# CVMI-Lab/HybridNeuralRendering

Hardware: AMD Instinct MI355X
Metric: rays/sec (fwd render) scene0241_01 at 1/2/4/8 GPU; PSNR delta vs ref (higher is better)
Workload: dtype f32

## Files before the change

### hybridneuralrendering_amd/csrc/mlp.hip

```cpp
#include <stdlib.h>

#include "hnr_h2.h"
#include "hnr_launch.h"

namespace hnr {

constexpr int ML_PAD = 32;
constexpr int ML_SLOT = 8192 + ML_PAD;
constexpr int ML_WSTEP = 8192;
constexpr int ML_META_FLOATS = 4 * 128 + 4 + 4;
constexpr int ML_DESC = 4 * 128, ML_WMAX = 4 * 128 + 4;

struct MlpArgs {
    const float *A; int lda;
    const float *R; const int32_t *ridx; int ldr;
    const char *wimg;
    int wbase[4];
    int K0, N[4], act[4];
    float *C2; int ldc2;
    const float *loc_w; const int32_t *vs_item;
    const float *w2c, *Kmat, *campos, *campos_n;
    const float *fm; int H, W;
    const float *frame_w;
    const float *w_last, *b_last;
    const float *CF; int ldcf;
    float *X7; int ld7;
    float slope;
    const unsigned long long *counts; int count_index, count_mult; long long M_cap;
    int seg_stride;
    float *C; int ldc;
    float *T0; int ldt0; float *T1; int ldt1;
    unsigned *tmax;
};

typedef float f32x4m __attribute__((ext_vector_type(4)));

#ifdef HNR_MLP_PROBE
__device__ long long g_mlp_probe[24];
#define MLP_STAMP(i_) do { const long long t_ = clock64(); tm_[i_] += t_ - tp_; tp_ = t_; if ((i_) == 0) ++ntile_; } while (0)
#else
#define MLP_STAMP(i_) do { } while (0)
#endif
constexpr int mlp3_wgs_per_cu(int S0, int RT, int MODE) { return MODE == 1 ? (RT >= 4 ? 2 : 4) : RT >= 4 ? 1 : (RT == 1 || S0 <= 6) ? 4 : 2; }

#ifdef HNR_MLP_FULL_BARRIER
#define MLP_LDS_BARRIER() __syncthreads()
#else
#define MLP_LDS_BARRIER() asm volatile("s_waitcnt lgkmcnt(0)\n\ts_barrier" ::: "memory")
#endif
#ifndef HNR_MLP_LPR16
#define HNR_MLP_LPR16 1
#endif
template <int S0, int S1, int S2, int S3, int MODE, int RT = 4>
__global__ __launch_bounds__(256, mlp3_wgs_per_cu(S0, RT, MODE)) void mlp3_kernel(MlpArgs a)
{
    static_assert(MODE != 1 || RT == 4 || RT == 2, "the merge stage is built on 128- or 64-row tiles (32 / 16 samples x 4 views)");
    constexpr int SLOT = RT * 2048 + ML_PAD, ROWS = 32 * RT;
    constexpr int SMAX3 = S0 > S1 ? (S0 > S2 ? S0 : S2) : (S1 > S2 ? S1 : S2), SMAX = SMAX3 > S3 ? SMAX3 : S3;
    extern __shared__ __attribute__((aligned(16))) char lds[];
    const int tid = threadIdx.x, lane = tid & 63, wave = tid >> 6, h = lane >> 5, j = lane & 31;
    long long M = a.M_cap;
    if (a.counts) { const long long c = (long long)a.counts[a.count_index] * a.count_mult; if (c < M) M = c; }
    long long n_unit = 1;
    if (a.seg_stride > 0) {
        n_unit = a.counts ? (long long)a.counts[a.count_index] : a.M_cap / (a.count_mult > 0 ? a.count_mult : 1);
        if (n_unit > a.seg_stride) n_unit = a.seg_stride;
        if (n_unit < 1) n_unit = 1;
        if (M > n_unit * a.count_mult) M = n_unit * a.count_mult;
    }
    auto phys = [&](long long m) -> long long {
        if (a.seg_stride <= 0) return m;
        int q = 0;
        for (int v = 1; v < a.count_mult && v < 8; ++v) q += (m >= (long long)v * n_unit) ? 1 : 0;
        return (long long)q * a.seg_stride + (m - (long long)q * n_unit);
    };
    const int n_tiles = (int)((M + ROWS - 1) / ROWS);
    const int total_steps = S0 + S1 + S2 + S3;
    const float *meta = reinterpret_cast<const float *>(a.wimg + (size_t)total_steps * ML_WSTEP);
    const __amdgpu_buffer_rsrc_t wsrd = __builtin_amdgcn_make_buffer_rsrc(const_cast<char *>(a.wimg), 0, total_steps * ML_WSTEP, 0x00020000);
    float *exch = reinterpret_cast<float *>(lds + SMAX * SLOT);
    float *rowinv = exch + ROWS * 4;
    float *s_f = rowinv + ROWS;
    int *s_pix = reinterpret_cast<int *>(s_f + ROWS * 48);
    float *s_vm = reinterpret_cast<float *>(s_pix + ROWS), *s_w = s_vm + ROWS;
    float *s_wl = s_w + ROWS;
    constexpr bool RS = S1 <= 4 && S2 <= 4 && S3 == 0 && RT >= 2;
    constexpr int RTW = RS ? RT / 2 : RT;
    const int cw = RS ? (wave & 1) : wave, rt0 = RS ? (wave >> 1) * RTW : 0;
    const int col0 = 32 * cw + 16 * h;
    const unsigned woff = (unsigned)cw * 2048u + (unsigned)lane * 16u;
    const char *lds_b = lds + rt0 * 2048;
    const f32x2 slope2 = {a.slope, a.slope};

    if (MODE == 1) {
        for (int i = tid; i < 128; i += 256) s_wl[i] = i < a.N[2] ? a.w_last[i] : 0.f;
    }
    float tmax_run[3] = {0.f, 0.f, 0.f};
#ifdef HNR_MLP_PROBE
    long long tm_[20] = {0, 0, 0, 0, 0, 0, 0, 0, 0, 0, 0, 0, 0, 0, 0, 0, 0, 0, 0, 0}, tp_ = clock64(), ntile_ = 0;
#endif
    for (int tile = blockIdx.x; tile < n_tiles; tile += gridDim.x) {
        const long long row_base = (long long)tile * ROWS;
        int tid_t = tid;
        asm volatile("" : "+v"(tid_t));
        MLP_STAMP(0);
        float inv[RTW];
        if (MODE == 1) {
            if (tid < 2 * ROWS) {
                const int row_t = tid % ROWS, ls = row_t >> 2, v = row_t & 3;
                long long sidx = row_base / 4 + ls;
                if (sidx * 4 >= M) sidx = M / 4 - 1;
                const float *pw = a.loc_w + (size_t)a.vs_item[sidx] * 3;
                const float x = pw[0], y = pw[1], z = pw[2];
              if (tid < ROWS) {
                int px, py;
                const bool inval = hnr_project_pixel(x, y, z, a.w2c + 16 * v, a.Kmat, a.W, a.H, px, py);
                s_pix[tid] = ((v * a.H + py) * a.W + px) * 48;
                s_vm[tid] = inval ? 0.f : 1.f;
              } else {
                const float cx = x - a.campos[0], cy = y - a.campos[1], cz = z - a.campos[2];
                const float cn = sqrtf(cx * cx + cy * cy + cz * cz) + 1e-6f;
                const float nx = x - a.campos_n[3 * v], ny = y - a.campos_n[3 * v + 1], nz = z - a.campos_n[3 * v + 2];
                const float nn = sqrtf(nx * nx + ny * ny + nz * nz) + 1e-6f;
                s_f[row_t * 48 + 45] = hnr_div(nx, nn) - hnr_div(cx, cn); s_f[row_t * 48 + 46] = hnr_div(ny, nn) - hnr_div(cy, cn); s_f[row_t * 48 + 47] = hnr_div(nz, nn) - hnr_div(cz, cn);
              }
            }
            MLP_STAMP(13);
            __syncthreads();
            {
                constexpr int NF = ROWS * 12 / 256;
                float4 f4[NF];
#pragma unroll
                for (int it = 0; it < NF; ++it) {
                    const int idx = tid_t + 256 * it, row = idx / 12, q = idx - row * 12;
                    f4[it] = *reinterpret_cast<const float4 *>(a.fm + (size_t)s_pix[row] + 4 * q);
                }
#pragma unroll
                for (int it = 0; it < NF; ++it) {
                    const int idx = tid_t + 256 * it, row = idx / 12, q = idx - row * 12;
                    float *d = s_f + row * 48 + 4 * q;
                    if (q < 11) *reinterpret_cast<float4 *>(d) = f4[it]; else d[0] = f4[it].x;
                }
            }
            __syncthreads();
            if (wave < RT) {
                const float *src = s_f + (32 * wave + j) * 48 + 8 * h;
                float x[3][8];
                float m = 0.f;
#pragma unroll
                for (int s = 0; s < 3; ++s) {
                    const float4 v0 = *reinterpret_cast<const float4 *>(src + 16 * s), v1 = *reinterpret_cast<const float4 *>(src + 16 * s + 4);
                    const float t[8] = {v0.x, v0.y, v0.z, v0.w, v1.x, v1.y, v1.z, v1.w};
#pragma unroll
                    for (int e = 0; e < 8; ++e) { x[s][e] = t[e]; m = fmaxf(m, fabsf(t[e])); }
                }
                m = fmaxf(m, __shfl_xor(m, 32));
                const int k = row_scale_exp(m);
                const float sc = pow2f(k);
                if (h == 0) rowinv[32 * wave + j] = pow2f(-k);
#pragma unroll
                for (int s = 0; s < 3; ++s) {
                    unsigned ph[4], pm[4];
#pragma unroll
                    for (int q = 0; q < 4; ++q) split2h(__fmul_rn(x[s][2 * q], sc), __fmul_rn(x[s][2 * q + 1], sc), ph[q], pm[q]);
                    char *dst = lds + s * SLOT + (wave * 2) * 1024 + lane * 16;
                    *reinterpret_cast<u32x4 *>(dst) = u32x4{ph[0], ph[1], ph[2], ph[3]};
                    *reinterpret_cast<u32x4 *>(dst + 1024) = u32x4{pm[0], pm[1], pm[2], pm[3]};
                }
            }
        } else
        {
            constexpr int COLS = 16 * S0, LPR = HNR_MLP_LPR16 && COLS == 288 ? 16 : (COLS > 128 ? 64 : (COLS > 64 ? 32 : 16)), RPI = 64 / LPR, NB = (COLS + 4 * LPR - 1) / (4 * LPR);
            const int lr = lane % LPR, sub = lane / LPR;
            constexpr int RW = 8 * RT;
            constexpr int ROWS_B = ((RW / RPI) * NB * 4 <= (RT < 4 ? 128 : 256)) ? RW : RW / 2;
            constexpr int BATCH = ROWS_B / RPI;
#pragma unroll 1
            for (int r0 = 0; r0 < RW; r0 += ROWS_B) {
                float4 v[BATCH][NB];
#pragma unroll
                for (int b = 0; b < BATCH; ++b) {
                    const int rl = RW * wave + r0 + b * RPI + sub;
                    long long row = row_base + rl;
                    if (row >= M) row = M - 1;
                    const float *src = a.A + (size_t)phys(row) * a.lda;
#pragma unroll
                    for (int nb = 0; nb < NB; ++nb) {
                        const int c = 4 * (nb * LPR + lr);
                        v[b][nb] = *reinterpret_cast<const float4 *>(src + (c + 4 <= a.lda ? c : 0));
                    }
                }
#pragma unroll
                for (int b = 0; b < BATCH; ++b) {
                    const int rl = RW * wave + r0 + b * RPI + sub;
                    float m = 0.f;
#pragma unroll
                    for (int nb = 0; nb < NB; ++nb) {
                        const int c = 4 * (nb * LPR + lr);
                        float *t = reinterpret_cast<float *>(&v[b][nb]);
#pragma unroll
                        for (int e = 0; e < 4; ++e) { t[e] = (c + e < a.K0) ? t[e] : 0.f; m = fmaxf(m, fabsf(t[e])); }
                    }
                    m = fmaxf(m, __builtin_amdgcn_update_dpp(m, m, 0xB1, 0xf, 0xf, false));
                    m = fmaxf(m, __builtin_amdgcn_update_dpp(m, m, 0x4E, 0xf, 0xf, false));
                    m = fmaxf(m, __builtin_amdgcn_update_dpp(m, m, 0x141, 0xf, 0xf, false));
                    m = fmaxf(m, __builtin_amdgcn_update_dpp(m, m, 0x140, 0xf, 0xf, false));
                    if (LPR >= 32) m = fmaxf(m, __builtin_amdgcn_update_dpp(m, m, 0x142, 0xa, 0xf, false));
                    if (LPR >= 64) m = fmaxf(m, __builtin_amdgcn_update_dpp(m, m, 0x143, 0xc, 0xf, false));
                    if (LPR == 64) m = __int_as_float(__builtin_amdgcn_readlane(__float_as_int(m), 63));
                    else if (LPR == 32) { const float m0 = __int_as_float(__builtin_amdgcn_readlane(__float_as_int(m), 31)), m1 = __int_as_float(__builtin_amdgcn_readlane(__float_as_int(m), 63)); m = sub ? m1 : m0; }
                    const int k = row_scale_exp(m);
                    const float sc = pow2f(k);
                    if (lr == 0) rowinv[rl] = pow2f(-k);
#pragma unroll
                    for (int nb = 0; nb < NB; ++nb) {
                        const int c = 4 * (nb * LPR + lr);
                        if (c < COLS) {
                            unsigned ph0, pm0, ph1, pm1;
                            split2h(__fmul_rn(v[b][nb].x, sc), __fmul_rn(v[b][nb].y, sc), ph0, pm0);
                            split2h(__fmul_rn(v[b][nb].z, sc), __fmul_rn(v[b][nb].w, sc), ph1, pm1);
                            char *dst = lds + (c >> 4) * SLOT + ((rl >> 5) * 2) * 1024 + ((((c >> 3) & 1) * 32 + (rl & 31)) * 16) + (c & 7) * 2;
                            *reinterpret_cast<uint2 *>(dst) = make_uint2(ph0, ph1);
                            *reinterpret_cast<uint2 *>(dst + 1024) = make_uint2(pm0, pm1);
                        }
                    }
                }
            }
        }
        MLP_STAMP(1);
        __syncthreads();
        MLP_STAMP(2);
        {
            const float dw0 = meta[ML_DESC + 0];
#pragma unroll
            for (int rt = 0; rt < RTW; ++rt) inv[rt] = __fmul_rn(rowinv[32 * (rt0 + rt) + j], dw0);
        }

        f32x16 acc[RTW][1];
        auto zero_acc = [&]() {
#pragma unroll
            for (int rt = 0; rt < RTW; ++rt)
#pragma unroll
                for (int r = 0; r < 16; ++r) acc[rt][0][r] = 0.f;
        };
        float4 ad[2][4];
        auto load_addend = [&](int rt) {
            long long row = row_base + 32 * (rt0 + rt) + j;
            if (row >= M) row = M - 1;
            const float *rrow = a.R + (size_t)(MODE == 1 ? row / 4 : (long long)a.ridx[phys(row)]) * a.ldr + col0;
#pragma unroll
            for (int q4 = 0; q4 < 4; ++q4) ad[rt & 1][q4] = *reinterpret_cast<const float4 *>(rrow + 4 * q4);
        };
        auto activate = [&](int layer, float (&amax)[RTW], auto with_addend) {
            constexpr bool ADD = decltype(with_addend)::value;
            f32x2 bias[8];
#pragma unroll
            for (int q = 0; q < 4; ++q) {
                const float4 b = *reinterpret_cast<const float4 *>(meta + layer * 128 + col0 + 4 * q);
                bias[2 * q] = f32x2{b.x, b.y}; bias[2 * q + 1] = f32x2{b.z, b.w};
            }
            const bool act = a.act[layer] != 0;
            if (ADD && MODE != 1) { load_addend(0); if (RTW > 1) load_addend(1); }
#pragma unroll
            for (int rt = 0; rt < RTW; ++rt) {
                float m = 0.f;
                const f32x2 inv2 = {inv[rt], inv[rt]};
#pragma unroll
                for (int q = 0; q < 8; ++q) {
                    f32x2 add = bias[q];
                    if (ADD) { const float4 t4 = ad[rt & 1][q >> 1]; add = add + ((q & 1) ? f32x2{t4.z, t4.w} : f32x2{t4.x, t4.y}); }
                    f32x2 v = f32x2_fma(f32x2{acc[rt][0][2 * q], acc[rt][0][2 * q + 1]}, inv2, add);
                    if (act) { const f32x2 sv = v * slope2; v.x = fmaxf(v.x, sv.x); v.y = fmaxf(v.y, sv.y); }
                    acc[rt][0][2 * q] = v.x; acc[rt][0][2 * q + 1] = v.y;
                    m = fmaxf(fmaxf(m, fabsf(v.x)), fabsf(v.y));
                }
                amax[rt] = m;
                if (ADD && rt + 2 < RTW) load_addend(rt + 2);
            }
        };
        auto publish = [&](int next_layer, bool active, float (&amax)[RTW]) {
#pragma unroll
            for (int rt = 0; rt < RTW; ++rt) {
                const float m = active ? fmaxf(amax[rt], __shfl_xor(amax[rt], 32)) : 0.f;
                if (h == 0) exch[(32 * (rt0 + rt) + j) * 4 + cw] = m;
            }
            __syncthreads();
            const float dw = meta[ML_DESC + next_layer];
#pragma unroll
            for (int rt = 0; rt < RTW; ++rt) {
                float4 m4 = *reinterpret_cast<const float4 *>(exch + (32 * (rt0 + rt) + j) * 4);
                if (RS) { m4.z = 0.f; m4.w = 0.f; }
                const int k = row_scale_exp(fmaxf(fmaxf(m4.x, m4.y), fmaxf(m4.z, m4.w)));
                const float sc = pow2f(k);
                const f32x2 sc2 = {sc, sc};
                inv[rt] = __fmul_rn(pow2f(-k), dw);
                if (active) {
                    unsigned ph[8], pm[8];
#pragma unroll
                    for (int q = 0; q < 8; ++q) {
                        const f32x2 vs = f32x2{acc[rt][0][2 * q], acc[rt][0][2 * q + 1]} * sc2;
                        split2h(vs.x, vs.y, ph[q], pm[q]);
                    }
                    char *dst = lds + (2 * cw + h) * SLOT + ((rt0 + rt) * 2) * 1024 + j * 16;
                    *reinterpret_cast<u32x4 *>(dst) = u32x4{ph[0], ph[1], ph[2], ph[3]};
                    *reinterpret_cast<u32x4 *>(dst + 512) = u32x4{ph[4], ph[5], ph[6], ph[7]};
                    *reinterpret_cast<u32x4 *>(dst + 1024) = u32x4{pm[0], pm[1], pm[2], pm[3]};
                    *reinterpret_cast<u32x4 *>(dst + 1024 + 512) = u32x4{pm[4], pm[5], pm[6], pm[7]};
                }
            }
            __syncthreads();
        };
        auto store = [&](float *C, int ldc) {
#pragma unroll
            for (int rt = 0; rt < RTW; ++rt) {
                const long long row = row_base + 32 * (rt0 + rt) + j;
                if (row < M) {
                    float *o = C + (size_t)phys(row) * ldc + col0;
#pragma unroll
                    for (int q = 0; q < 4; ++q) {
                        const int c = col0 + 4 * q;
                        if (c + 4 <= ldc)
                            *reinterpret_cast<float4 *>(o + 4 * q) = make_float4(acc[rt][0][4 * q], acc[rt][0][4 * q + 1], acc[rt][0][4 * q + 2], acc[rt][0][4 * q + 3]);
                    }
                }
            }
        };
        const bool act0 = 32 * cw < a.N[0], act1 = 32 * cw < a.N[1], act2 = 32 * cw < a.N[2];
        float amax[RTW];
        zero_acc();
        if (act0) {
            h2_mfma_layer<RTW, 1, S0, 0, ML_WSTEP, SLOT>(wsrd, a.wbase[0], woff, lds_b, lane, acc, []() {}, [&]() { if (MODE == 1) { load_addend(0); load_addend(1); } });
            MLP_STAMP(3);
            if (a.R) activate(0, amax, std::true_type{}); else activate(0, amax, std::false_type{});
            MLP_STAMP(4);
            if (MODE == 0 && a.T0) {
                store(a.T0, a.ldt0);
#pragma unroll
                for (int rt = 0; rt < RTW; ++rt) tmax_run[0] = fmaxf(tmax_run[0], amax[rt]);
            }
        }
        publish(1, act0, amax);
        MLP_STAMP(5);
        zero_acc();
        if (act1) {
            h2_mfma_layer<RTW, 1, S1, 0, ML_WSTEP, SLOT>(wsrd, a.wbase[1], woff, lds_b, lane, acc, []() {});
            MLP_STAMP(6);
            activate(1, amax, std::false_type{});
            if (MODE == 0 && a.T1) {
                store(a.T1, a.ldt1);
#pragma unroll
                for (int rt = 0; rt < RTW; ++rt) tmax_run[1] = fmaxf(tmax_run[1], amax[rt]);
            }
        }
        publish(2, act1, amax);
        MLP_STAMP(7);
        float cfv[6] = {0.f, 0.f, 0.f, 0.f, 0.f, 0.f};
        float4 wl4[4];
        zero_acc();
        if (act2) {
            h2_mfma_layer<RTW, 1, S2, 0, ML_WSTEP, SLOT>(wsrd, a.wbase[2], woff, lds_b, lane, acc, []() {});
            MLP_STAMP(8);
            activate(2, amax, std::false_type{});
            MLP_STAMP(9);
            if (MODE != 1) store(a.C, a.ldc);
            if (MODE == 0 && a.tmax) {
#pragma unroll
                for (int rt = 0; rt < RTW; ++rt) tmax_run[2] = fmaxf(tmax_run[2], amax[rt]);
            }
            MLP_STAMP(10);
        }
        if (MODE == 1) {
#pragma unroll
            for (int it = 0; it < (8 * RT * 45 + 255) / 256; ++it) {
                const int idx = tid_t + 256 * it, ls = idx / 45, ch = idx - ls * 45;
                const long long sidx = row_base / 4 + ls;
                cfv[it] = (idx < 8 * RT * 45 && sidx * 4 < M) ? a.CF[(size_t)sidx * a.ldcf + ch] : 0.f;
            }
#pragma unroll
            for (int q4 = 0; q4 < 4; ++q4) wl4[q4] = *reinterpret_cast<const float4 *>(s_wl + col0 + 4 * q4);
        }
        if (MODE == 1) {
#pragma unroll
            for (int rt = 0; rt < RTW; ++rt) {
                float d = 0.f;
                if (act2) {
#pragma unroll
                    for (int r = 0; r < 16; ++r) d = fmaf(acc[rt][0][r], reinterpret_cast<const float *>(wl4)[r], d);
                    d = __fadd_rn(d, __shfl_xor(d, 32));
                }
                if (h == 0) exch[(32 * (rt0 + rt) + j) * 4 + cw] = d;
            }
            MLP_LDS_BARRIER();
            MLP_STAMP(14);
            if (tid < ROWS) {
                float4 d4 = *reinterpret_cast<const float4 *>(exch + tid * 4);
                if (RS) { d4.z = 0.f; d4.w = 0.f; }
                const float d = __fadd_rn(__fadd_rn(d4.x, d4.y), __fadd_rn(d4.z, d4.w));
                float wv = hnr_div(1.f, 1.f + expf(-(d + a.b_last[0])));
                wv *= s_vm[tid];
                if (a.frame_w) wv *= a.frame_w[tid & 3];
                s_w[tid] = wv;
            }
            MLP_LDS_BARRIER();
            MLP_STAMP(15);
            {
#pragma unroll
                for (int it = 0; it < (8 * RT * 45 + 255) / 256; ++it) {
                    const int idx = tid_t + 256 * it, ls = idx / 45, ch = idx - ls * 45;
                    const long long sidx = row_base / 4 + ls;
                    if (idx < 8 * RT * 45 && sidx * 4 < M) {
                        float fsum = 0.f, wsum = 0.f;
#pragma unroll
                        for (int v = 0; v < 4; ++v) { const float wv = s_w[4 * ls + v]; fsum += s_f[(4 * ls + v) * 48 + ch] * wv; wsum += wv; }
                        float *o = a.X7 + (size_t)sidx * a.ld7;
                        __builtin_nontemporal_store(cfv[it], o + ch);
                        __builtin_nontemporal_store(hnr_div(fsum, wsum + 1e-6f), o + 45 + ch);
                    }
                }
                MLP_STAMP(17);
            }
        }
        if (S3 > 0) {
            publish(3, act2, amax);
            zero_acc();
            if (32 * wave < a.N[3]) {
                h2_mfma_layer<RTW, 1, (S3 > 0 ? S3 : 1), 0, ML_WSTEP, SLOT>(wsrd, a.wbase[3], woff, lds_b, lane, acc, []() {});
                activate(3, amax, std::false_type{});
                store(a.C2, a.ldc2);
            }
        }
        MLP_STAMP(11);
        __syncthreads();
        MLP_STAMP(12);
    }
    if (MODE == 0 && a.tmax) {
        __syncthreads();
#pragma unroll
        for (int l = 0; l < 3; ++l) {
            float m = tmax_run[l];
            for (int o = 32; o > 0; o >>= 1) m = fmaxf(m, __shfl_xor(m, o));
            if (lane == 0) exch[4 * l + wave] = m;
        }
        __syncthreads();
        if (tid < 3) { const float m = fmaxf(fmaxf(exch[4 * tid], exch[4 * tid + 1]), fmaxf(exch[4 * tid + 2], exch[4 * tid + 3])); if (m > 0.f) atomicMax(a.tmax + tid, __float_as_uint(m)); }
    }
#ifdef HNR_MLP_PROBE
    if (blockIdx.x == 0 && threadIdx.x == 0) { for (int i = 0; i < 20; ++i) g_mlp_probe[i] = tm_[i]; g_mlp_probe[20] = ntile_; }
#endif
}

constexpr int MW_SLOT = 2048 + ML_PAD;
constexpr int MW_WAVE_LDS = 4 * MW_SLOT + 4 * 32 * 4 + 32 * 3 * 4;
constexpr int MW_WAVES = 12;
constexpr int MW_WBYTES = 11 * 4096;
constexpr int MW_SHARED = MW_WBYTES + 3 * 64 * 4 + 64 * 4 + 128 * 4;
constexpr int MW_LDS = MW_SHARED + MW_WAVES * MW_WAVE_LDS;
#define MW_WAVE_FENCE() asm volatile("s_waitcnt lgkmcnt(0)" ::: "memory")
template <int S>
__device__ __forceinline__ void mw_layer(const char *wp, const char *bp, f32x16 (&acc)[2])
{
    u32x4 wf[2][2][2], bf[2][2];
    auto ld = [&](int slot, int s) {
#pragma unroll
        for (int c = 0; c < 2; ++c)
#pragma unroll
            for (int q = 0; q < 2; ++q) wf[slot][c][q] = *reinterpret_cast<const u32x4 *>(wp + s * 4096 + (c * 2 + q) * 1024);
#pragma unroll
        for (int q = 0; q < 2; ++q) bf[slot][q] = *reinterpret_cast<const u32x4 *>(bp + s * MW_SLOT + q * 1024);
    };
    ld(0, 0);
#pragma unroll
    for (int s = 0; s < S; ++s) {
        if (s + 1 < S) ld((s + 1) & 1, s + 1);
        const int b = s & 1;
#define MW_W(c, q) __builtin_bit_cast(f16x8, wf[b][c][q])
#define MW_X(q) __builtin_bit_cast(f16x8, bf[b][q])
#pragma unroll
        for (int c = 0; c < 2; ++c) acc[c] = __builtin_amdgcn_mfma_f32_32x32x16_f16(MW_W(c, 1), MW_X(0), acc[c], 0, 0, 0);
#pragma unroll
        for (int c = 0; c < 2; ++c) acc[c] = __builtin_amdgcn_mfma_f32_32x32x16_f16(MW_W(c, 0), MW_X(1), acc[c], 0, 0, 0);
#pragma unroll
        for (int c = 0; c < 2; ++c) acc[c] = __builtin_amdgcn_mfma_f32_32x32x16_f16(MW_W(c, 0), MW_X(0), acc[c], 0, 0, 0);
#undef MW_W
#undef MW_X
    }
}

__global__ __launch_bounds__(64 * MW_WAVES, 1) void merge_wp_kernel(MlpArgs a)
{
    extern __shared__ __attribute__((aligned(16))) char lds[];
    const int tid = threadIdx.x, wave = __builtin_amdgcn_readfirstlane(tid >> 6);
    long long M = a.M_cap;
    if (a.counts) { const long long c = (long long)a.counts[a.count_index] * a.count_mult; if (c < M) M = c; }
    const long long n_samp = M / 4;
    const int n_tiles = (int)((n_samp + 7) / 8);
    const float *meta = reinterpret_cast<const float *>(a.wimg + (size_t)11 * ML_WSTEP);
    float *s_bias = reinterpret_cast<float *>(lds + MW_WBYTES);
    float *s_wl = s_bias + 3 * 64;
    float *s_cam = s_wl + 64;
    char *wl = lds + MW_SHARED + wave * MW_WAVE_LDS;
    int *s_pix = reinterpret_cast<int *>(wl + 4 * MW_SLOT);
    float *s_vm = reinterpret_cast<float *>(s_pix + 32), *s_w = s_vm + 32;
    unsigned *s_max = reinterpret_cast<unsigned *>(s_w + 32);
    float *s_dd = reinterpret_cast<float *>(s_max + 32);
    for (int i = tid; i < MW_WBYTES / 16; i += 64 * MW_WAVES) {
        const int s = i >> 8, cp = (i >> 6) & 3, ln = i & 63;
        *reinterpret_cast<u32x4 *>(lds + i * 16) = *reinterpret_cast<const u32x4 *>(a.wimg + (size_t)s * ML_WSTEP + cp * 1024 + ln * 16);
    }
    for (int i = tid; i < 3 * 64; i += 64 * MW_WAVES) s_bias[i] = meta[(i >> 6) * 128 + (i & 63)];
    for (int i = tid; i < 64; i += 64 * MW_WAVES) { s_wl[i] = a.w_last[i]; s_cam[i] = a.w2c[i]; }
    if (tid < 9) s_cam[64 + tid] = a.Kmat[tid];
    if (tid < 3) s_cam[76 + tid] = a.campos[tid];
    if (tid < 12) s_cam[80 + tid] = a.campos_n[tid];
    __syncthreads();
    const float dw0 = meta[ML_DESC + 0], dw1 = meta[ML_DESC + 1], dw2 = meta[ML_DESC + 2], b_last = a.b_last[0];
    const f32x2 slope2 = {a.slope, a.slope};
    for (int tile = blockIdx.x * MW_WAVES + wave; tile < n_tiles; tile += gridDim.x * MW_WAVES) {
        int lane = tid & 63;
        asm volatile("" : "+v"(lane));
        const int h = lane >> 5, j = lane & 31;
        const long long sbase = (long long)tile * 8;
        {
            const int ls = j >> 2, v = j & 3;
            long long sidx = sbase + ls;
            if (sidx >= n_samp) sidx = n_samp - 1;
            const float *pw = a.loc_w + (size_t)a.vs_item[sidx] * 3;
            const float x = pw[0], y = pw[1], z = pw[2];
            if (h == 0) {
                int px, py;
                const bool inval = hnr_project_pixel(x, y, z, s_cam + 16 * v, s_cam + 64, a.W, a.H, px, py);
                s_pix[j] = ((v * a.H + py) * a.W + px) * 48;
                s_vm[j] = inval ? 0.f : 1.f;
                s_max[j] = 0u;
            } else {
                const float *cp = s_cam + 76, *cnp = s_cam + 80 + 3 * v;
                const float cx = x - cp[0], cy = y - cp[1], cz = z - cp[2];
                const float cn = sqrtf(cx * cx + cy * cy + cz * cz) + 1e-6f;
                const float nx = x - cnp[0], ny = y - cnp[1], nz = z - cnp[2];
                const float nn = sqrtf(nx * nx + ny * ny + nz * nz) + 1e-6f;
                s_dd[j * 3] = hnr_div(nx, nn) - hnr_div(cx, cn); s_dd[j * 3 + 1] = hnr_div(ny, nn) - hnr_div(cy, cn); s_dd[j * 3 + 2] = hnr_div(nz, nn) - hnr_div(cz, cn);
            }
        }
        MW_WAVE_FENCE();
        float inv;
        {
            float4 f4[6];
#pragma unroll
            for (int it = 0; it < 6; ++it) {
                const int idx = lane + 64 * it, row = idx / 12, q = idx - row * 12;
                f4[it] = *reinterpret_cast<const float4 *>(a.fm + (size_t)s_pix[row] + 4 * q);
            }
#pragma unroll
            for (int it = 0; it < 6; ++it) {
                const int idx = lane + 64 * it, row = idx / 12, q = idx - row * 12;
                if (q == 11) { f4[it].y = s_dd[row * 3]; f4[it].z = s_dd[row * 3 + 1]; f4[it].w = s_dd[row * 3 + 2]; }
                const float m = fmaxf(fmaxf(fabsf(f4[it].x), fabsf(f4[it].y)), fmaxf(fabsf(f4[it].z), fabsf(f4[it].w)));
                atomicMax(s_max + row, __float_as_uint(m));
            }
            MW_WAVE_FENCE();
#pragma unroll
            for (int it = 0; it < 6; ++it) {
                const int idx = lane + 64 * it, row = idx / 12, q = idx - row * 12, c = 4 * q;
                const float sc = pow2f(row_scale_exp(__uint_as_float(s_max[row])));
                unsigned ph0, pm0, ph1, pm1;
                split2h(__fmul_rn(f4[it].x, sc), __fmul_rn(f4[it].y, sc), ph0, pm0);
                split2h(__fmul_rn(f4[it].z, sc), __fmul_rn(f4[it].w, sc), ph1, pm1);
                char *dst = wl + (c >> 4) * MW_SLOT + ((((c >> 3) & 1) * 32 + row) * 16) + (c & 7) * 2;
                *reinterpret_cast<uint2 *>(dst) = make_uint2(ph0, ph1);
                *reinterpret_cast<uint2 *>(dst + 1024) = make_uint2(pm0, pm1);
            }
            inv = __fmul_rn(pow2f(-row_scale_exp(__uint_as_float(s_max[j]))), dw0);
        }
        float4 ad[2][4];
        {
            long long sidx = sbase + (j >> 2);
            if (sidx >= n_samp) sidx = n_samp - 1;
            const float *rrow = a.R + (size_t)sidx * a.ldr + 16 * h;
#pragma unroll
            for (int c = 0; c < 2; ++c)
#pragma unroll
                for (int q4 = 0; q4 < 4; ++q4) ad[c][q4] = *reinterpret_cast<const float4 *>(rrow + 32 * c + 4 * q4);
        }
        MW_WAVE_FENCE();
        f32x16 acc[2];
        auto zero_acc = [&]() {
#pragma unroll
            for (int c = 0; c < 2; ++c)
#pragma unroll
                for (int r = 0; r < 16; ++r) acc[c][r] = 0.f;
        };
        auto activate = [&](int layer, auto with_addend) -> float {
            constexpr bool ADD = decltype(with_addend)::value;
            float m = 0.f;
            const f32x2 inv2 = {inv, inv};
#pragma unroll
            for (int c = 0; c < 2; ++c) {
#pragma unroll
                for (int q4 = 0; q4 < 4; ++q4) {
                    const float4 b = *reinterpret_cast<const float4 *>(s_bias + layer * 64 + 32 * c + 16 * h + 4 * q4);
#pragma unroll
                    for (int e = 0; e < 2; ++e) {
                        const int q = 2 * q4 + e;
                        f32x2 add = e ? f32x2{b.z, b.w} : f32x2{b.x, b.y};
                        if (ADD) { const float4 t4 = ad[c][q4]; add = add + (e ? f32x2{t4.z, t4.w} : f32x2{t4.x, t4.y}); }
                        f32x2 v = f32x2_fma(f32x2{acc[c][2 * q], acc[c][2 * q + 1]}, inv2, add);
                        const f32x2 sv = v * slope2;
                        v.x = fmaxf(v.x, sv.x); v.y = fmaxf(v.y, sv.y);
                        acc[c][2 * q] = v.x; acc[c][2 * q + 1] = v.y;
                        m = fmaxf(fmaxf(m, fabsf(v.x)), fabsf(v.y));
                    }
                }
            }
            return m;
        };
        auto publish = [&](float dw, float m) {
            m = fmaxf(m, __shfl_xor(m, 32));
            const int k = row_scale_exp(m);
            const float sc = pow2f(k);
            const f32x2 sc2 = {sc, sc};
            inv = __fmul_rn(pow2f(-k), dw);
            MW_WAVE_FENCE();
#pragma unroll
            for (int c = 0; c < 2; ++c) {
                unsigned ph[8], pm[8];
#pragma unroll
                for (int q = 0; q < 8; ++q) {
// ... 554 lines not shown
```

Before: 8.092 million.

## Transpose MLP output stores across lane quads and skip interior column masking

```diff
diff --git a/hybridneuralrendering_amd/csrc/mlp.hip b/hybridneuralrendering_amd/csrc/mlp.hip
--- a/hybridneuralrendering_amd/csrc/mlp.hip
+++ b/hybridneuralrendering_amd/csrc/mlp.hip
@@ -51,6 +51,25 @@
 #ifndef HNR_MLP_LPR16
 #define HNR_MLP_LPR16 1
 #endif
+template <int X> __device__ __forceinline__ float ml_quad_xor(float v)
+{
+    static_assert(X >= 1 && X <= 3, "lane t ^ X of a quad");
+    constexpr int ctrl = X == 1 ? 0xB1 : X == 2 ? 0x4E : 0x1B;
+    return __builtin_bit_cast(float, __builtin_amdgcn_update_dpp(0, __builtin_bit_cast(int, v), ctrl, 0xf, 0xf, true));
+}
+__device__ __forceinline__ void ml_quad_swap(float4 &r0, float4 &r1, float4 &r2, float4 &r3)
+{
+    unsigned long long keep;
+    asm volatile("s_mov_b64 %16, exec\n\ts_mov_b32 exec_lo, 0xaaaaaaaa\n\ts_mov_b32 exec_hi, 0xaaaaaaaa\n\t"
+                 "v_swap_b32 %0, %4\n\tv_swap_b32 %1, %5\n\tv_swap_b32 %2, %6\n\tv_swap_b32 %3, %7\n\t"
+                 "v_swap_b32 %8, %12\n\tv_swap_b32 %9, %13\n\tv_swap_b32 %10, %14\n\tv_swap_b32 %11, %15\n\t"
+                 "s_mov_b32 exec_lo, 0xcccccccc\n\ts_mov_b32 exec_hi, 0xcccccccc\n\t"
+                 "v_swap_b32 %0, %8\n\tv_swap_b32 %1, %9\n\tv_swap_b32 %2, %10\n\tv_swap_b32 %3, %11\n\t"
+                 "v_swap_b32 %4, %12\n\tv_swap_b32 %5, %13\n\tv_swap_b32 %6, %14\n\tv_swap_b32 %7, %15\n\t"
+                 "s_mov_b64 exec, %16\n\ts_nop 1"
+                 : "+v"(r0.x), "+v"(r0.y), "+v"(r0.z), "+v"(r0.w), "+v"(r1.x), "+v"(r1.y), "+v"(r1.z), "+v"(r1.w),
+                   "+v"(r2.x), "+v"(r2.y), "+v"(r2.z), "+v"(r2.w), "+v"(r3.x), "+v"(r3.y), "+v"(r3.z), "+v"(r3.w), "=&s"(keep));
+}
 template <int S0, int S1, int S2, int S3, int MODE, int RT = 4>
 __global__ __launch_bounds__(256, mlp3_wgs_per_cu(S0, RT, MODE)) void mlp3_kernel(MlpArgs a)
 {
@@ -68,10 +87,15 @@
         if (n_unit < 1) n_unit = 1;
         if (M > n_unit * a.count_mult) M = n_unit * a.count_mult;
     }
+    auto seg_of = [&](long long m) -> int {
+        int q = 0;
+        if (a.seg_stride > 0)
+            for (int v = 1; v < a.count_mult && v < 8; ++v) q += (m >= (long long)v * n_unit) ? 1 : 0;
+        return q;
+    };
     auto phys = [&](long long m) -> long long {
         if (a.seg_stride <= 0) return m;
-        int q = 0;
-        for (int v = 1; v < a.count_mult && v < 8; ++v) q += (m >= (long long)v * n_unit) ? 1 : 0;
+        const int q = seg_of(m);
         return (long long)q * a.seg_stride + (m - (long long)q * n_unit);
     };
     const int n_tiles = (int)((M + ROWS - 1) / ROWS);
@@ -175,6 +199,7 @@
             constexpr int RW = 8 * RT;
             constexpr int ROWS_B = ((RW / RPI) * NB * 4 <= (RT < 4 ? 128 : 256)) ? RW : RW / 2;
             constexpr int BATCH = ROWS_B / RPI;
+            auto edge = [](int nb) { return 4 * LPR * (nb + 1) > COLS - 16; };
 #pragma unroll 1
             for (int r0 = 0; r0 < RW; r0 += ROWS_B) {
                 float4 v[BATCH][NB];
@@ -187,7 +212,7 @@
 #pragma unroll
                     for (int nb = 0; nb < NB; ++nb) {
                         const int c = 4 * (nb * LPR + lr);
-                        v[b][nb] = *reinterpret_cast<const float4 *>(src + (c + 4 <= a.lda ? c : 0));
+                        v[b][nb] = *reinterpret_cast<const float4 *>(src + (!edge(nb) || c + 4 <= a.lda ? c : 0));
                     }
                 }
 #pragma unroll
@@ -199,7 +224,7 @@
                         const int c = 4 * (nb * LPR + lr);
                         float *t = reinterpret_cast<float *>(&v[b][nb]);
 #pragma unroll
-                        for (int e = 0; e < 4; ++e) { t[e] = (c + e < a.K0) ? t[e] : 0.f; m = fmaxf(m, fabsf(t[e])); }
+                        for (int e = 0; e < 4; ++e) { if (edge(nb)) t[e] = (c + e < a.K0) ? t[e] : 0.f; m = fmaxf(m, fabsf(t[e])); }
                     }
                     m = fmaxf(m, __builtin_amdgcn_update_dpp(m, m, 0xB1, 0xf, 0xf, false));
                     m = fmaxf(m, __builtin_amdgcn_update_dpp(m, m, 0x4E, 0xf, 0xf, false));
@@ -311,17 +336,35 @@
             __syncthreads();
         };
         auto store = [&](float *C, int ldc) {
+            int jl = j, c0 = col0;
+            asm volatile("" : "+v"(jl), "+v"(c0));
+            const int t = jl & 3, pmax = ((ldc - c0) >> 2) - 1;
 #pragma unroll
             for (int rt = 0; rt < RTW; ++rt) {
-                const long long row = row_base + 32 * (rt0 + rt) + j;
-                if (row < M) {
-                    float *o = C + (size_t)phys(row) * ldc + col0;
-#pragma unroll
-                    for (int q = 0; q < 4; ++q) {
-                        const int c = col0 + 4 * q;
-                        if (c + 4 <= ldc)
-                            *reinterpret_cast<float4 *>(o + 4 * q) = make_float4(acc[rt][0][4 * q], acc[rt][0][4 * q + 1], acc[rt][0][4 * q + 2], acc[rt][0][4 * q + 3]);
+                const f32x16 &v = acc[rt][0];
+                float4 tb[4];
+                tb[0] = make_float4(v[0], v[1], v[2], v[3]);
+                tb[1] = make_float4(ml_quad_xor<1>(v[4]), ml_quad_xor<1>(v[5]), ml_quad_xor<1>(v[6]), ml_quad_xor<1>(v[7]));
+                tb[2] = make_float4(ml_quad_xor<2>(v[8]), ml_quad_xor<2>(v[9]), ml_quad_xor<2>(v[10]), ml_quad_xor<2>(v[11]));
+                tb[3] = make_float4(ml_quad_xor<3>(v[12]), ml_quad_xor<3>(v[13]), ml_quad_xor<3>(v[14]), ml_quad_xor<3>(v[15]));
+                ml_quad_swap(tb[0], tb[1], tb[2], tb[3]);
+                const long long row0 = row_base + 32 * (rt0 + rt) + (jl & ~3), left = M - row0;
+                const int nrow = left >= 4 ? 4 : left > 0 ? (int)left : 0;
+                const int q0 = seg_of(row0);
+                const long long rel = row0 - (long long)q0 * n_unit;
+                float *o = C + (size_t)((long long)q0 * a.seg_stride + rel) * ldc + c0;
+                if (a.seg_stride > 0) {
+                    const long long rem = n_unit - rel, gap = (long long)a.seg_stride - n_unit;
+                    const int remc = rem < 8 ? (int)rem : 8, nuc = n_unit < 8 ? (int)n_unit : 8;
+#pragma unroll
+                    for (int r = 0; r < 4; ++r) {
+                        const int k = (r >= remc ? 1 : 0) + (r >= remc + nuc ? 1 : 0) + (r >= remc + 2 * nuc ? 1 : 0);
+                        if (r < nrow && (r ^ t) <= pmax) *reinterpret_cast<float4 *>(o + (size_t)(r + k * gap) * ldc + 4 * (r ^ t)) = tb[r];
                     }
+                } else {
+#pragma unroll
+                    for (int r = 0; r < 4; ++r)
+                        if (r < nrow && (r ^ t) <= pmax) *reinterpret_cast<float4 *>(o + (size_t)r * ldc + 4 * (r ^ t)) = tb[r];
                 }
             }
         };
```

Result: no change. 8.110 million, median of 6 (+0.2%).
